# Wells-Group/pmg-dolfinx

Measured on NVIDIA B200. Metric: fine-level Gdof/s per p-MG V-cycle (P4->P2->P1, Chebyshev(2), CSR coarse solve), higher is better.
Workload: dtype f64

## Files before the change

pmg_dolfinx_b200/csrc/amg.cu:

```cuda
#include "common.hpp"
#include "operator.hpp"
#include "csr.hpp"
#include "solvers.hpp"
#include "amg.hpp"

#include <algorithm>
#include <cstdlib>
#include <cstring>

namespace pmgx
{
namespace
{
__global__ void __launch_bounds__(256)
k_dense_rows(int n_rows, int n_cols, const double* __restrict__ inv, const double* __restrict__ b,
             double* __restrict__ x)
{
  const int row = (blockIdx.x * blockDim.x + threadIdx.x) >> 5, lane = threadIdx.x & 31;
  if (row >= n_rows)
    return;
  const double* r = inv + (size_t)row * n_cols;
  double s = 0.0;
  for (int c = lane; c < n_cols; c += 32)
    s = fma(r[c], b[c], s);
#pragma unroll
  for (int o = 16; o > 0; o >>= 1)
    s += __shfl_xor_sync(0xffffffffu, s, o);
  if (lane == 0)
    x[row] = s;
}

__global__ void k_permute(int n, const int32_t* __restrict__ perm, const double* __restrict__ in, double* __restrict__ out)
{
  const int g = blockIdx.x * blockDim.x + threadIdx.x;
  if (g < n)
    out[g] = in[perm[g]];
}

struct RectSell
{
  int n_rows = 0;
  DevBuf<long long> slice_ptr;
  DevBuf<int32_t> cols;
  DevBuf<double> vals;
  void upload(const amg::Csr& M, cudaStream_t st)
  {
    n_rows = M.n_rows;
    const int ns = (n_rows + 31) / 32;
    std::vector<long long> sp((size_t)ns + 1, 0);
    for (int s = 0; s < ns; ++s)
    {
      int w = 0;
      for (int r = s * 32; r < std::min(n_rows, s * 32 + 32); ++r)
        w = std::max(w, (int)(M.ptr[r + 1] - M.ptr[r]));
      sp[s + 1] = sp[s] + (long long)w * 32;
    }
    std::vector<int32_t> c((size_t)std::max<long long>(sp[ns], 1), 0);
    std::vector<double> v((size_t)std::max<long long>(sp[ns], 1), 0.0);
    for (int r = 0; r < n_rows; ++r)
      for (int32_t j = M.ptr[r], k = 0; j < M.ptr[r + 1]; ++j, ++k)
      {
        const size_t p = (size_t)sp[r >> 5] + (size_t)k * 32 + (r & 31);
        c[p] = M.cols[j];
        v[p] = M.vals[j];
      }
    slice_ptr.upload(sp.data(), sp.size(), st);
    cols.upload(c.data(), c.size(), st);
    vals.upload(v.data(), v.size(), st);
  }
};

struct RectCsr
{
  int n_rows = 0;
  DevBuf<int32_t> ptr, cols;
  DevBuf<double> vals;
  void upload(const amg::Csr& M, cudaStream_t st)
  {
    n_rows = M.n_rows;
    ptr.upload(M.ptr.data(), M.ptr.size(), st);
    cols.upload(M.cols.data(), M.cols.size(), st);
    vals.upload(M.vals.data(), M.vals.size(), st);
  }
};

pmgx_halo* make_halo(pmgx_ctx* c, int n_owned, int n_ghost, const amg::Plan& p)
{
  if (c->nranks == 1)
    return nullptr;
  pmgx_halo* h = nullptr;
  const int rc = pmgx_halo_create(c, n_owned, n_ghost, (int)p.send_ranks.size(), p.send_ranks.data(), p.send_offsets.data(),
                                  p.send_idx.data(), (int)p.recv_ranks.size(), p.recv_ranks.data(), p.recv_offsets.data(),
                                  p.recv_idx.data(), &h);
  if (rc != PMGX_OK)
    throw Error{rc};
  static const bool ss = !(getenv("PMGX_AMG_SINGLE_STREAM") && atoi(getenv("PMGX_AMG_SINGLE_STREAM")) == 0);
  h->single_stream = ss && h->p2p && h->n_send() + h->n_recv() <= 65536;
  return h;
}

struct AmgPrecond : Precond
{
  struct Lv
  {
    int n_owned = 0, n_ghost = 0;
    long long nnz = 0;
    pmgx_operator* A = nullptr;
    bool own_A = false;
    pmgx_operator* A_lp = nullptr;
    pmgx_halo* halo = nullptr;
    pmgx_halo* halo_v = nullptr;
    pmgx_cheb* sm = nullptr;
    RectCsr R;
    RectSell P;
    DevBuf<double> x, b;
    DevBuf<double> x2, r2;
    long long nnz_p = 0;
    bool dense = false;
    int n_global = 0;
    DevBuf<double> inv;
    pmgx_halo* gather = nullptr;
    bool repl_first = false;
    int n_mine = 0;
    pmgx_halo* repl_gather = nullptr;
    DevBuf<double> bg;
    DevBuf<int32_t> perm;
  };
  pmgx_ctx* ctx = nullptr;
  std::vector<Lv> lv;
  int nu = 2;
  int gamma = 1;
  int gamma_from = 0;

  ~AmgPrecond() override
  {
    for (Lv& L : lv)
    {
      if (L.sm)
        pmgx_cheb_destroy(L.sm);
      if (L.A_lp)
        pmgx_operator_destroy(L.A_lp);
      if (L.own_A && L.A)
        pmgx_operator_destroy(L.A);
      if (L.halo)
        pmgx_halo_destroy(L.halo);
      if (L.gather)
        pmgx_halo_destroy(L.gather);
      if (L.repl_gather)
        pmgx_halo_destroy(L.repl_gather);
    }
  }

  void cycle(int l, const double* b, double* x)
  {
    Lv& L = lv[l];
    if (l + 1 == (int)lv.size())
    {
      if (L.dense)
      {
        double* bb = L.b.p;
        if (b != bb)
          vec::copy(ctx, bb, b, L.n_owned);
        if (L.gather)
        {
          halo_fwd_begin(L.gather, bb);
          halo_fwd_end(L.gather, bb);
        }
        if (L.n_owned > 0)
        {
          k_dense_rows<<<(L.n_owned * 32 + 255) / 256, 256, 0, ctx->stream>>>(L.n_owned, L.n_global, L.inv.p, bb, x);
          check_launch("k_dense_rows");
          count_launch(ctx);
        }
      }
      else
        cheb_solve(L.sm, L.A, x, b, nullptr, true, CHEB_R_NONE);
      return;
    }
    Lv& C = lv[l + 1];
    pmgx_operator* As = L.A_lp ? L.A_lp : L.A;
    cheb_solve(L.sm, As, x, b, nullptr, true, CHEB_R_FULL);
    if (L.halo_v)
    {
      halo_fwd_begin(L.halo_v, L.sm->r.p);
      halo_fwd_end(L.halo_v, L.sm->r.p);
    }
    if (C.repl_first)
    {
      spmv_rect(ctx, C.n_mine, L.R.ptr.p, L.R.cols.p, L.R.vals.p, L.sm->r.p, C.bg.p, false, 32);
      halo_fwd_begin(C.repl_gather, C.bg.p);
      halo_fwd_end(C.repl_gather, C.bg.p);
      k_permute<<<(C.n_owned + 255) / 256, 256, 0, ctx->stream>>>(C.n_owned, C.perm.p, C.bg.p, C.b.p);
      check_launch("k_permute");
      count_launch(ctx);
    }
    else
      spmv_rect(ctx, C.n_owned, L.R.ptr.p, L.R.cols.p, L.R.vals.p, L.sm->r.p, C.b.p, false, 32);
    cycle(l + 1, C.b.p, C.x.p);
    if (gamma == 2 && l >= gamma_from && l + 2 < (int)lv.size())
    {
      C.A->apply(C.x.p, C.r2.p);
      vec::axpy(ctx, C.r2.p, -1.0, C.r2.p, C.b.p, C.n_owned);
      cycle(l + 1, C.r2.p, C.x2.p);
      vec::axpy(ctx, C.x.p, 1.0, C.x2.p, C.x.p, C.n_owned);
    }
    if (C.halo_v)
    {
      halo_fwd_begin(C.halo_v, C.x.p);
      halo_fwd_end(C.halo_v, C.x.p);
    }
    spmv_sell_rect(ctx, L.n_owned, L.P.slice_ptr.p, L.P.cols.p, L.P.vals.p, C.x.p, x, true);
    cheb_solve(L.sm, As, x, b, nullptr, false, CHEB_R_NONE);
  }

  void apply(const double* r, double* u) override { cycle(0, r, u); }
};

amg::Plan plan_of(pmgx_halo* h)
{
  amg::Plan p;
  if (!h)
    return p;
  p.send_ranks = h->send_ranks;
  p.send_offsets = h->send_offsets;
  p.recv_ranks = h->recv_ranks;
  p.recv_offsets = h->recv_offsets;
  if (p.send_offsets.empty())
    p.send_offsets.assign(1, 0);
  if (p.recv_offsets.empty())
    p.recv_offsets.assign(1, 0);
  p.send_idx.resize((size_t)h->n_send());
  p.recv_idx.resize((size_t)h->n_recv());
  if (!p.send_idx.empty())
    PMGX_CUDA(cudaMemcpy(p.send_idx.data(), h->send_idx.p, p.send_idx.size() * sizeof(int32_t), cudaMemcpyDeviceToHost));
  if (!p.recv_idx.empty())
    PMGX_CUDA(cudaMemcpy(p.recv_idx.data(), h->recv_idx.p, p.recv_idx.size() * sizeof(int32_t), cudaMemcpyDeviceToHost));
  return p;
}
}
}

using pmgx::AmgPrecond;

extern "C"
{
int pmgx_coarse_create_amg(pmgx_ctx* ctx, pmgx_operator* A, int max_iter, double rtol, int nu, int min_coarse,
                           int max_levels, pmgx_coarse** out)
{
  PMGX_API_BEGIN
  PMGX_REQUIRE(ctx && A && out && max_iter >= 0, "coarse_create_amg: bad arguments");
  PMGX_REQUIRE(A->kind == pmgx_operator::CSR, "coarse_create_amg: the operator must be an assembled CSR operator");
  PMGX_REQUIRE(nu >= 1 && nu <= 8, "coarse_create_amg: nu must be in 1..8");
  PMGX_CUDA(cudaSetDevice(ctx->device));
  if (min_coarse <= 0)
    min_coarse = 600;
  if (max_levels <= 0)
    max_levels = 12;
  auto* Ac = static_cast<pmgx::CsrOperator*>(A);
  PMGX_REQUIRE(ctx->nranks == 1 || Ac->halo || Ac->n_ghost == 0, "coarse_create_amg: the operator has ghosts but no halo");
  pmgx::amg::Csr A0;
  A0.ptr.resize((size_t)Ac->n_owned + 1);
  A0.cols.resize((size_t)Ac->nnz);
  A0.vals.resize((size_t)Ac->nnz);
  {
    const int rc = pmgx_csr_get(A, A0.ptr.data(), A0.cols.data(), A0.vals.data());
    if (rc != PMGX_OK)
      return rc;
    std::vector<std::pair<int32_t, double>> row;
    for (int i = 0; i < Ac->n_owned; ++i)
    {
      bool sorted = true;
      for (int32_t j = A0.ptr[i] + 1; j < A0.ptr[i + 1] && sorted; ++j)
        sorted = A0.cols[j - 1] < A0.cols[j];
      if (sorted)
        continue;
      row.clear();
      for (int32_t j = A0.ptr[i]; j < A0.ptr[i + 1]; ++j)
        row.emplace_back(A0.cols[j], A0.vals[j]);
      std::sort(row.begin(), row.end());
      for (size_t t = 0; t < row.size(); ++t)
        A0.cols[A0.ptr[i] + t] = row[t].first, A0.vals[A0.ptr[i] + t] = row[t].second;
    }
  }
  pmgx::amg::Csr Az;
  if (getenv("PMGX_AMG_DROP_ZEROS") && atoi(getenv("PMGX_AMG_DROP_ZEROS")) == 1 && Ac->n_owned > 0)
  {
    A0.n_rows = Ac->n_owned;
    A0.n_cols = Ac->n_owned + Ac->n_ghost;
    Az = pmgx::amg::drop_stored_zeros(A0);
    if (Az.nnz() * 5 > A0.nnz() * 4)
      Az = pmgx::amg::Csr();
  }
  const pmgx::amg::Plan plan0 = pmgx::plan_of(Ac->halo);
  pmgx::amg::Comm cm;
  cm.rank = ctx->rank;
  cm.nranks = ctx->nranks;
  cm.allgather = [ctx](const void* mine, size_t bytes, void* all)
  {
    std::vector<char> buf;
    pmgx::p2p::allgather_bytes(ctx, mine, bytes, buf);
    std::memcpy(all, buf.data(), bytes * (size_t)ctx->nranks);
  };
  pmgx::amg::Hierarchy H;
  pmgx::amg::setup(H, std::move(A0), Ac->n_owned, Ac->n_ghost, plan0, cm, min_coarse, max_levels);

  std::unique_ptr<AmgPrecond> M(new AmgPrecond());
  M->ctx = ctx;
  M->nu = nu;
  int nu_coarse = nu;
  if (const char* e = getenv("PMGX_AMG_NU_COARSE"))
    nu_coarse = std::min(std::max(atoi(e), 1), 8);
  if (const char* e = getenv("PMGX_AMG_GAMMA"))
    M->gamma = atoi(e) == 2 ? 2 : 1;
  if (const char* e = getenv("PMGX_AMG_GAMMA_FROM"))
    M->gamma_from = std::max(atoi(e), 0);
  const bool use_lp = !(getenv("PMGX_AMG_LP") && atoi(getenv("PMGX_AMG_LP")) == 0);
  const int fuse_from = getenv("PMGX_AMG_FUSE_FROM") ? atoi(getenv("PMGX_AMG_FUSE_FROM")) : 1;
  const int nl = (int)H.levels.size();
  M->lv.resize((size_t)nl);
  for (int l = 0; l < nl; ++l)
  {
    pmgx::amg::Level& L = H.levels[l];
    AmgPrecond::Lv& D = M->lv[l];
    D.n_owned = L.n_owned;
    D.n_ghost = L.n_ghost;
    D.nnz = L.A.nnz();
    const bool last = l + 1 == nl;
    if (l == 0)
    {
      D.A = A;
      D.halo_v = Ac->halo;
      if (!Az.ptr.empty())
      {
        std::vector<int32_t> off((size_t)Ac->n_owned);
        for (int i = 0; i < Ac->n_owned; ++i)
        {
          int32_t j = Az.ptr[i];
          while (j < Az.ptr[i + 1] && Az.cols[j] < Ac->n_owned)
            ++j;
          off[i] = j;
        }
        pmgx_operator* Acmp = nullptr;
        const int rc = pmgx_csr_create(ctx, Ac->n_owned, Ac->n_ghost, Az.ptr.data(), off.data(), Az.cols.data(),
                                       Az.vals.data(), Ac->halo, &Acmp);
        if (rc != PMGX_OK)
          return rc;
        D.A = Acmp;
        D.own_A = true;
      }
    }
    else
    {
      if (!L.replicated)
      {
        D.halo = pmgx::make_halo(ctx, L.n_owned, L.n_ghost, L.plan);
        D.halo_v = D.halo;
      }
      else if (L.n_mine > 0 || !L.gather_perm.empty())
      {
        D.repl_first = true;
        D.n_mine = L.n_mine;
        D.repl_gather = pmgx::make_halo(ctx, L.n_mine, L.n_owned - L.n_mine, L.repl_plan);
        D.bg.alloc((size_t)std::max(L.n_owned, 1));
        PMGX_CUDA(cudaMemsetAsync(D.bg.p, 0, (size_t)std::max(L.n_owned, 1) * sizeof(double), ctx->stream));
        D.perm.upload(L.gather_perm.data(), L.gather_perm.size(), ctx->stream);
      }
      std::vector<int32_t> off((size_t)L.n_owned);
      for (int i = 0; i < L.n_owned; ++i)
      {
        int32_t j = L.A.ptr[i];
        while (j < L.A.ptr[i + 1] && L.A.cols[j] < L.n_owned)
          ++j;
        off[i] = j;
      }
      const int rc = pmgx_csr_create(ctx, L.n_owned, L.n_ghost, L.A.ptr.data(), off.data(), L.A.cols.data(),
                                     L.A.vals.data(), D.halo, &D.A);
      if (rc != PMGX_OK)
        return rc;
      D.own_A = true;
      const size_t nt = (size_t)L.n_owned + L.n_ghost;
      for (auto* buf : {&D.x, &D.b, &D.x2, &D.r2})
      {
        buf->alloc(nt);
        if (nt > 0)
          PMGX_CUDA(cudaMemsetAsync(buf->p, 0, nt * sizeof(double), ctx->stream));
      }
    }
    {
      const int rc = pmgx_cheb_create(ctx, L.n_owned, L.n_ghost, 0.1 * L.lmax, L.lmax, &D.sm);
      if (rc != PMGX_OK)
        return rc;
      D.sm->max_iter = (last && !L.dense) ? 4 * nu : (l == 0 ? nu : nu_coarse);
      D.sm->fuse = l >= fuse_from;
    }
    if (l == 0 && !last && use_lp)
      D.A_lp = pmgx::make_lp(static_cast<pmgx::CsrOperator*>(D.A));
    D.nnz_p = L.P.nnz();
    if (!last)
    {
      D.P.upload(L.P, ctx->stream);
      D.R.upload(L.R, ctx->stream);
    }
    else if (L.dense)
    {
      D.dense = true;
      D.n_global = (int)L.n_global;
      D.inv.upload(L.inv_rows.data(), L.inv_rows.size(), ctx->stream);
      const int n_gather = (int)L.n_global - L.n_owned;
      if (!L.replicated)
        D.gather = pmgx::make_halo(ctx, L.n_owned, n_gather, L.gather_plan);
      const size_t nt = (size_t)L.n_owned + std::max(L.n_ghost, n_gather);
      D.b.alloc(nt);
      if (nt > 0)
        PMGX_CUDA(cudaMemsetAsync(D.b.p, 0, nt * sizeof(double), ctx->stream));
    }
  }
  PMGX_CUDA(cudaStreamSynchronize(ctx->stream));

  pmgx_coarse* cs = nullptr;
  const int rc = pmgx_coarse_create(ctx, M->lv[0].A, max_iter, rtol, &cs);
  if (rc != PMGX_OK)
    return rc;
  cs->M = M.release();
  cs->check_every = 1;
  if (const char* e = getenv("PMGX_COARSE_CHECK_EVERY"))
    cs->check_every = std::max(atoi(e), 1);
  *out = cs;
  PMGX_API_END
}

int pmgx_coarse_num_levels(pmgx_coarse* cs)
{
  if (!cs)
    return -1;
  return cs->M ? (int)static_cast<AmgPrecond*>(cs->M)->lv.size() : 1;
}

int pmgx_coarse_level_info(pmgx_coarse* cs, int level, long long* out_h)
{
  PMGX_API_BEGIN
  PMGX_REQUIRE(cs && out_h && level >= 0 && level < pmgx_coarse_num_levels(cs), "coarse_level_info: bad arguments");
  if (!cs->M)
  {
    out_h[0] = cs->A->n_owned;
    out_h[1] = pmgx_csr_nnz(cs->A);
    out_h[2] = cs->A->n_ghost;
    out_h[3] = 0;
    out_h[4] = 0;
  }
  else
  {
    const AmgPrecond::Lv& L = static_cast<AmgPrecond*>(cs->M)->lv[level];
    out_h[0] = L.n_owned;
    out_h[1] = L.nnz;
    out_h[2] = L.n_ghost;
    out_h[3] = L.dense ? 1 : 0;
    out_h[4] = L.nnz_p;
  }
  PMGX_API_END
}

int pmgx_coarse_apply_preconditioner(pmgx_coarse* cs, const double* r, double* u)
{
  PMGX_API_BEGIN
  PMGX_REQUIRE(cs && r && u && r != u, "coarse_apply_preconditioner: bad arguments");
  PMGX_CUDA(cudaSetDevice(cs->ctx->device));
  if (cs->M)
    cs->M->apply(r, u);
  else
    pmgx::vec::pointwise_mult(cs->ctx, u, r, cs->A->diag_inv.p, cs->A->n_owned);
  PMGX_API_END
}
}
```

pmg_dolfinx_b200/csrc/csr.cu:

```cuda
#include "common.hpp"
#include "operator.hpp"
#include "csr.hpp"
#include "solvers.hpp"

namespace pmgx
{
namespace
{
constexpr int LPR = 8;
constexpr int ST = 256;

constexpr int UNR = 4;
template <bool ACCUM>
__global__ void __launch_bounds__(ST)
k_spmv(int n_rows, const double* __restrict__ vals, const int32_t* __restrict__ beg,
       const int32_t* __restrict__ end, const int32_t* __restrict__ cols,
       const double* __restrict__ x, double* __restrict__ y)
{
  const int gt = blockIdx.x * blockDim.x + threadIdx.x;
  const int row = gt / LPR, lane = gt % LPR;
  double s = 0.0;
  if (row < n_rows)
  {
    const int e = end[row];
    for (int j0 = beg[row] + lane; j0 < e; j0 += UNR * LPR)
    {
      int c[UNR];
      double v[UNR];
#pragma unroll
      for (int t = 0; t < UNR; ++t)
      {
        const int jj = j0 + t * LPR;
        const bool ok = jj < e;
        c[t] = ok ? __ldcs(cols + jj) : -1;
        v[t] = ok ? __ldcs(vals + jj) : 0.0;
      }
#pragma unroll
      for (int t = 0; t < UNR; ++t)
        if (c[t] >= 0)
          s = fma(v[t], x[c[t]], s);
    }
  }
#pragma unroll
  for (int o = LPR / 2; o > 0; o >>= 1)
    s += __shfl_xor_sync(0xffffffffu, s, o);
  if (row < n_rows && lane == 0)
    y[row] = ACCUM ? y[row] + s : s;
}

__global__ void __launch_bounds__(ST)
k_spmv_ghost_rows(int n_list, const int32_t* __restrict__ rows, const double* __restrict__ vals,
                  const int32_t* __restrict__ off_diag, const int32_t* __restrict__ row_ptr,
                  const int32_t* __restrict__ cols, const double* __restrict__ x, double* __restrict__ y)
{
  const int gt = blockIdx.x * blockDim.x + threadIdx.x;
  const int li = gt / LPR, lane = gt % LPR;
  double s = 0.0;
  int row = -1;
  if (li < n_list)
  {
    row = rows[li];
    const int e = row_ptr[row + 1];
    for (int j = off_diag[row] + lane; j < e; j += LPR)
      s = fma(vals[j], x[cols[j]], s);
  }
#pragma unroll
  for (int o = LPR / 2; o > 0; o >>= 1)
    s += __shfl_xor_sync(0xffffffffu, s, o);
  if (row >= 0 && lane == 0)
    y[row] += s;
}

template <int MODE>
__device__ __forceinline__ void cheb_row(int i, double q, const double* __restrict__ in, const ChebEp& e)
{
  if (MODE == ChebEp::INIT)
  {
    const double rv = q * (-1.0) + e.b[i];
    e.r[i] = rv;
    e.z_out[i] = (rv * e.dinv[i]) * e.c0;
  }
  else if (MODE == ChebEp::LAST)
    e.r[i] = q * (-1.0) + e.r[i];
  else
  {
    const double rv = q * (-1.0) + e.r[i];
    const double zo = in[i];
    const double zs = zo * e.c1;
    const double zv = (rv * e.dinv[i]) * e.c2 + zs;
    if (MODE == ChebEp::STEP)
    {
      e.r[i] = rv;
      e.z_out[i] = zv;
    }
    const double xo = e.defer == 2 ? zo : (e.defer == 1 ? zo * 1.0 + e.x[i] : e.x[i]);
    e.x[i] = zv * 1.0 + xo;
  }
}

template <typename VT, bool D16, int MODE>
__global__ void __launch_bounds__(ST)
k_spmv_cheb(int n_rows, const VT* __restrict__ vals, const int32_t* __restrict__ beg, const int32_t* __restrict__ end,
            const int32_t* __restrict__ row_ptr, const int16_t* __restrict__ dcol, const int32_t* __restrict__ cols,
            const double* __restrict__ x, const ChebEp e)
{
  const int gt = blockIdx.x * blockDim.x + threadIdx.x;
  const int row = gt / LPR, lane = gt % LPR;
  double s = 0.0;
  if (row < n_rows)
  {
    const int en = end[row];
    for (int j0 = beg[row] + lane; j0 < en; j0 += UNR * LPR)
    {
      int c[UNR];
      VT v[UNR];
#pragma unroll
      for (int t = 0; t < UNR; ++t)
      {
        const int jj = j0 + t * LPR;
        const bool ok = jj < en;
        c[t] = ok ? (D16 ? row + (int)__ldcs(dcol + jj) : __ldcs(cols + jj)) : -1;
        v[t] = ok ? __ldcs(vals + jj) : VT(0);
      }
#pragma unroll
      for (int t = 0; t < UNR; ++t)
        if (c[t] >= 0)
          s = fma((double)v[t], x[c[t]], s);
    }
  }
#pragma unroll
  for (int o = LPR / 2; o > 0; o >>= 1)
    s += __shfl_xor_sync(0xffffffffu, s, o);
  __shared__ double sq[ST / LPR];
  if (lane == 0)
    sq[threadIdx.x / LPR] = s;
  __syncthreads();
  if (threadIdx.x < ST / LPR)
  {
    const int r = blockIdx.x * (ST / LPR) + threadIdx.x;
    if (r < n_rows)
    {
      if (end[r] < row_ptr[r + 1])
        e.scratch[r] = sq[threadIdx.x];
      else
        cheb_row<MODE>(r, sq[threadIdx.x], x, e);
    }
  }
}

template <int MODE>
__global__ void __launch_bounds__(ST)
k_spmv_cheb_ghost_rows(int n_list, const int32_t* __restrict__ rows, const double* __restrict__ vals,
                       const int32_t* __restrict__ off_diag, const int32_t* __restrict__ row_ptr,
                       const int32_t* __restrict__ cols, const double* __restrict__ x, const ChebEp e)
{
  const int gt = blockIdx.x * blockDim.x + threadIdx.x;
  const int li = gt / LPR, lane = gt % LPR;
  double s = 0.0;
  int row = -1;
  if (li < n_list)
  {
    row = rows[li];
    const int en = row_ptr[row + 1];
    for (int j = off_diag[row] + lane; j < en; j += LPR)
      s = fma(vals[j], x[cols[j]], s);
  }
#pragma unroll
  for (int o = LPR / 2; o > 0; o >>= 1)
    s += __shfl_xor_sync(0xffffffffu, s, o);
  if (row >= 0 && lane == 0)
    cheb_row<MODE>(row, e.scratch[row] + s, x, e);
}

template <typename VT, bool D16>
void launch_spmv_cheb(pmgx_ctx* c, int grid, int n_rows, const VT* vals, const int32_t* beg, const int32_t* end,
                      const int32_t* row_ptr, const int16_t* dcol, const int32_t* cols, const double* x, const ChebEp& e)
{
  switch (e.mode)
  {
  case ChebEp::INIT: k_spmv_cheb<VT, D16, ChebEp::INIT><<<grid, ST, 0, c->stream>>>(n_rows, vals, beg, end, row_ptr, dcol, cols, x, e); break;
  case ChebEp::STEP: k_spmv_cheb<VT, D16, ChebEp::STEP><<<grid, ST, 0, c->stream>>>(n_rows, vals, beg, end, row_ptr, dcol, cols, x, e); break;
  case ChebEp::LAST: k_spmv_cheb<VT, D16, ChebEp::LAST><<<grid, ST, 0, c->stream>>>(n_rows, vals, beg, end, row_ptr, dcol, cols, x, e); break;
  default: k_spmv_cheb<VT, D16, ChebEp::XONLY><<<grid, ST, 0, c->stream>>>(n_rows, vals, beg, end, row_ptr, dcol, cols, x, e); break;
  }
  check_launch("k_spmv_cheb");
  count_launch(c);
}

void launch_ghost_rows_cheb(const CsrOperator* A, const double* x, const ChebEp& e)
{
  pmgx_ctx* c = A->ctx;
  const int g2 = (int)(((long long)A->n_ghost_rows * LPR + ST - 1) / ST);
#define PMGX_GR(M)                                                                                                     \
  k_spmv_cheb_ghost_rows<M><<<g2, ST, 0, c->stream>>>(A->n_ghost_rows, A->ghost_rows.p, A->values.p, A->off_diag.p,    \
                                                      A->row_ptr.p, A->cols.p, x, e)
  switch (e.mode)
  {
  case ChebEp::INIT: PMGX_GR(ChebEp::INIT); break;
  case ChebEp::STEP: PMGX_GR(ChebEp::STEP); break;
  case ChebEp::LAST: PMGX_GR(ChebEp::LAST); break;
  default: PMGX_GR(ChebEp::XONLY); break;
  }
#undef PMGX_GR
  check_launch("k_spmv_cheb_ghost_rows");
  count_launch(c);
}

__global__ void k_flag_ghost_rows(int n_rows, const int32_t* __restrict__ off_diag,
                                  const int32_t* __restrict__ row_ptr, int32_t* __restrict__ count,
                                  int32_t* __restrict__ list)
{
  const int i = blockIdx.x * blockDim.x + threadIdx.x;
  if (i < n_rows && off_diag[i] < row_ptr[i + 1])
    list[atomicAdd(count, 1)] = i;
}

__global__ void k_extract_diag_inv(int n_rows, const double* __restrict__ vals,
                                   const int32_t* __restrict__ row_ptr,
                                   const int32_t* __restrict__ cols, double* __restrict__ dinv)
{
  const int i = blockIdx.x * blockDim.x + threadIdx.x;
  if (i >= n_rows)
    return;
  double d = 0.0;
  for (int j = row_ptr[i]; j < row_ptr[i + 1]; ++j)
    if (cols[j] == i)
      d = 1.0 / vals[j];
  dinv[i] = d;
}

constexpr int SLICE = 32;

template <bool D16>
__global__ void __launch_bounds__(ST)
k_spmv_sell(int n_rows, const long long* __restrict__ slice_ptr, const float* __restrict__ vals,
            const int16_t* __restrict__ dcol, const int32_t* __restrict__ cols, const double* __restrict__ x,
            double* __restrict__ y)
{
  const int row = blockIdx.x * blockDim.x + threadIdx.x;
  const int s = row >> 5, lane = row & 31;
  if (s >= (n_rows + SLICE - 1) / SLICE)
    return;
  const long long b = slice_ptr[s];
  const int w = (int)((slice_ptr[s + 1] - b) >> 5);
  const float* v = vals + b + lane;
  const int16_t* d = dcol + b + lane;
  const int32_t* c = cols + b + lane;
  const int r = row < n_rows ? row : n_rows - 1;
  double s0 = 0.0, s1 = 0.0;
  int k = 0;
  for (; k + 4 <= w; k += 4)
  {
    float vv[4];
    int cc[4];
#pragma unroll
    for (int t = 0; t < 4; ++t)
    {
      vv[t] = __ldcs(v + (k + t) * SLICE);
      cc[t] = D16 ? r + (int)__ldcs(d + (k + t) * SLICE) : __ldcs(c + (k + t) * SLICE);
    }
    s0 = fma((double)vv[0], x[cc[0]], s0);
    s1 = fma((double)vv[1], x[cc[1]], s1);
    s0 = fma((double)vv[2], x[cc[2]], s0);
    s1 = fma((double)vv[3], x[cc[3]], s1);
  }
  for (; k < w; ++k)
  {
    const float vv = __ldcs(v + k * SLICE);
    const int cc = D16 ? r + (int)__ldcs(d + k * SLICE) : __ldcs(c + k * SLICE);
    s0 = fma((double)vv, x[cc], s0);
  }
  if (row < n_rows)
    y[row] = s0 + s1;
}

template <bool ACCUM>
__global__ void __launch_bounds__(ST)
k_spmv_sell_rect(int n_rows, const long long* __restrict__ slice_ptr, const double* __restrict__ vals,
                 const int32_t* __restrict__ cols, const double* __restrict__ x, double* __restrict__ y)
{
  const int row = blockIdx.x * blockDim.x + threadIdx.x;
  const int s = row >> 5, lane = row & 31;
  if (row >= n_rows)
    return;
  const long long b = slice_ptr[s];
  const int w = (int)((slice_ptr[s + 1] - b) >> 5);
  const double* v = vals + b + lane;
  const int32_t* c = cols + b + lane;
  double s0 = 0.0, s1 = 0.0;
  int k = 0;
  for (; k + 2 <= w; k += 2)
  {
    const double v0 = __ldcs(v + k * SLICE), v1 = __ldcs(v + (k + 1) * SLICE);
    const int c0 = __ldcs(c + k * SLICE), c1 = __ldcs(c + (k + 1) * SLICE);
    s0 = fma(v0, x[c0], s0);
    s1 = fma(v1, x[c1], s1);
  }
  if (k < w)
    s0 = fma(__ldcs(v + k * SLICE), x[__ldcs(c + k * SLICE)], s0);
  y[row] = ACCUM ? y[row] + (s0 + s1) : s0 + s1;
}

__global__ void k_sell_widths(int n_rows, const int32_t* __restrict__ row_ptr, const int32_t* __restrict__ off_diag,
                              const int32_t* __restrict__ cols, long long* __restrict__ widths, int* __restrict__ overflow)
{
  const int row = blockIdx.x * blockDim.x + threadIdx.x;
  int len = 0;
  bool ovf = false;
  if (row < n_rows)
  {
    len = off_diag[row] - row_ptr[row];
    for (int j = row_ptr[row]; j < off_diag[row]; ++j)
    {
      const int dlt = cols[j] - row;
      ovf = ovf || dlt > 32767 || dlt < -32767;
    }
  }
#pragma unroll
  for (int o = 16; o > 0; o >>= 1)
    len = max(len, __shfl_xor_sync(0xffffffffu, len, o));
  if (__any_sync(0xffffffffu, ovf) && (threadIdx.x & 31) == 0)
    atomicOr(overflow, 1);
  if ((threadIdx.x & 31) == 0 && row < n_rows)
    widths[row >> 5] = (long long)len * SLICE;
}

__global__ void k_sell_fill(int n_rows, const int32_t* __restrict__ row_ptr, const int32_t* __restrict__ off_diag,
                            const int32_t* __restrict__ cols, const double* __restrict__ vals,
                            const long long* __restrict__ slice_ptr, float* __restrict__ v32, int16_t* __restrict__ d16,
                            int32_t* __restrict__ c32)
{
  const int row = blockIdx.x * blockDim.x + threadIdx.x;
  const int s = row >> 5, lane = row & 31;
  if (s >= (n_rows + SLICE - 1) / SLICE)
    return;
  const long long b = slice_ptr[s];
  const int w = (int)((slice_ptr[s + 1] - b) >> 5);
  const int r = row < n_rows ? row : n_rows - 1;
  const int beg = row < n_rows ? row_ptr[row] : 0, len = row < n_rows ? off_diag[row] - row_ptr[row] : 0;
  for (int k = 0; k < w; ++k)
  {
    const long long p = b + (long long)k * SLICE + lane;
    const bool ok = k < len;
    v32[p] = ok ? (float)vals[beg + k] : 0.f;
    const int col = ok ? cols[beg + k] : r;
    if (d16)
      d16[p] = (int16_t)(col - r);
    if (c32)
      c32[p] = col;
  }
}

template <int LANES, bool ACCUM>
__global__ void __launch_bounds__(ST)
k_spmv_rect(int n_rows, const double* __restrict__ vals, const int32_t* __restrict__ ptr,
            const int32_t* __restrict__ cols, const double* __restrict__ x, double* __restrict__ y)
{
  const int gt = blockIdx.x * blockDim.x + threadIdx.x;
  const int row = gt / LANES, lane = gt % LANES;
  double s = 0.0;
  if (row < n_rows)
  {
    const int e = ptr[row + 1];
    for (int j = ptr[row] + lane; j < e; j += LANES)
      s = fma(vals[j], x[cols[j]], s);
  }
#pragma unroll
  for (int o = LANES / 2; o > 0; o >>= 1)
    s += __shfl_xor_sync(0xffffffffu, s, o);
  if (row < n_rows && lane == 0)
    y[row] = ACCUM ? y[row] + s : s;
}
}

void spmv_sell_rect(pmgx_ctx* c, int n_rows, const long long* slice_ptr, const int32_t* cols, const double* vals,
                    const double* x, double* y, bool accumulate)
{
  if (n_rows <= 0)
    return;
  const int grid = (n_rows + ST - 1) / ST;
  if (accumulate)
    k_spmv_sell_rect<true><<<grid, ST, 0, c->stream>>>(n_rows, slice_ptr, vals, cols, x, y);
  else
    k_spmv_sell_rect<false><<<grid, ST, 0, c->stream>>>(n_rows, slice_ptr, vals, cols, x, y);
  check_launch("k_spmv_sell_rect");
  count_launch(c);
}

void spmv_rect(pmgx_ctx* c, int n_rows, const int32_t* row_ptr, const int32_t* cols, const double* vals,
               const double* x, double* y, bool accumulate, int lanes)
{
  if (n_rows <= 0)
    return;
  const int grid = (int)(((long long)n_rows * lanes + ST - 1) / ST);
  if (lanes == 32)
  {
    if (accumulate)
      k_spmv_rect<32, true><<<grid, ST, 0, c->stream>>>(n_rows, vals, row_ptr, cols, x, y);
    else
      k_spmv_rect<32, false><<<grid, ST, 0, c->stream>>>(n_rows, vals, row_ptr, cols, x, y);
  }
  else if (lanes == 4)
  {
    if (accumulate)
      k_spmv_rect<4, true><<<grid, ST, 0, c->stream>>>(n_rows, vals, row_ptr, cols, x, y);
    else
      k_spmv_rect<4, false><<<grid, ST, 0, c->stream>>>(n_rows, vals, row_ptr, cols, x, y);
  }
  else
  {
    if (accumulate)
      k_spmv_rect<8, true><<<grid, ST, 0, c->stream>>>(n_rows, vals, row_ptr, cols, x, y);
    else
      k_spmv_rect<8, false><<<grid, ST, 0, c->stream>>>(n_rows, vals, row_ptr, cols, x, y);
  }
  check_launch("k_spmv_rect");
  count_launch(c);
}

void CsrOperator::apply(double* x, double* y)
{
  cudaSetDevice(ctx->device);
  const int grid = (int)(((long long)n_owned * LPR + ST - 1) / ST);
  if (n_ghost > 0)
    vec::set(ctx, y + n_owned, n_ghost, 0.0);
  if (halo)
    halo_fwd_begin(halo, x);
  if (n_owned > 0)
  {
    k_spmv<false><<<grid, ST, 0, ctx->stream>>>(n_owned, values.p, row_ptr.p, off_diag.p, cols.p, x, y);
    check_launch("k_spmv");
    count_launch(ctx);
  }
  if (halo)
    halo_fwd_end(halo, x);
  if (n_ghost_rows > 0)
  {
    const int g2 = (int)(((long long)n_ghost_rows * LPR + ST - 1) / ST);
    k_spmv_ghost_rows<<<g2, ST, 0, ctx->stream>>>(n_ghost_rows, ghost_rows.p, values.p, off_diag.p, row_ptr.p, cols.p,
                                                  x, y);
    check_launch("k_spmv_ghost_rows");
    count_launch(ctx);
  }
}

bool CsrOperator::apply_cheb(double* in, const ChebEp& e)
{
  cudaSetDevice(ctx->device);
  PMGX_REQUIRE(n_ghost_rows == 0 || e.scratch, "apply_cheb: scratch vector missing");
  const int grid = (int)(((long long)n_owned * LPR + ST - 1) / ST);
  if (halo)
    halo_fwd_begin(halo, in);
  if (n_owned > 0)
    launch_spmv_cheb<double, false>(ctx, grid, n_owned, values.p, row_ptr.p, off_diag.p, row_ptr.p, nullptr, cols.p, in, e);
  if (halo)
    halo_fwd_end(halo, in);
  if (n_ghost_rows > 0)
    launch_ghost_rows_cheb(this, in, e);
  return true;
}

void CsrOperatorLP::apply(double* x, double* y)
{
  cudaSetDevice(ctx->device);
  if (n_ghost > 0)
    vec::set(ctx, y + n_owned, n_ghost, 0.0);
  if (halo)
    halo_fwd_begin(halo, x);
  if (n_owned > 0)
  {
    const int grid = (n_slices * SLICE + ST - 1) / ST;
    if (d16)
      k_spmv_sell<true><<<grid, ST, 0, ctx->stream>>>(n_owned, slice_ptr.p, vals32.p, dcol16.p, nullptr, x, y);
    else
      k_spmv_sell<false><<<grid, ST, 0, ctx->stream>>>(n_owned, slice_ptr.p, vals32.p, nullptr, cols32.p, x, y);
    check_launch("k_spmv_sell");
    count_launch(ctx);
  }
  if (halo)
    halo_fwd_end(halo, x);
  if (src->n_ghost_rows > 0)
  {
    const int g2 = (int)(((long long)src->n_ghost_rows * LPR + ST - 1) / ST);
    k_spmv_ghost_rows<<<g2, ST, 0, ctx->stream>>>(src->n_ghost_rows, src->ghost_rows.p, src->values.p, src->off_diag.p,
                                                  src->row_ptr.p, src->cols.p, x, y);
    check_launch("k_spmv_ghost_rows");
    count_launch(ctx);
  }
}

CsrOperatorLP* make_lp(CsrOperator* A)
{
  pmgx_ctx* c = A->ctx;
  std::unique_ptr<CsrOperatorLP> L(new CsrOperatorLP());
  L->ctx = c;
  L->kind = pmgx_operator::CSR;
  L->n_owned = A->n_owned;
  L->n_ghost = A->n_ghost;
  L->halo = A->halo;
  L->src = A;
  L->diag_inv.alloc((size_t)A->n_owned);
  if (A->n_owned > 0)
    PMGX_CUDA(cudaMemcpyAsync(L->diag_inv.p, A->diag_inv.p, (size_t)A->n_owned * sizeof(double), cudaMemcpyDeviceToDevice, c->stream));
  const int n = A->n_owned;
  L->n_slices = (n + SLICE - 1) / SLICE;
  L->slice_ptr.alloc((size_t)L->n_slices + 1);
  PMGX_CUDA(cudaMemsetAsync(L->slice_ptr.p, 0, ((size_t)L->n_slices + 1) * sizeof(long long), c->stream));
  DevBuf<int> ovf;
  ovf.alloc(1);
  PMGX_CUDA(cudaMemsetAsync(ovf.p, 0, sizeof(int), c->stream));
  long long total = 0;
  if (n > 0)
  {
    k_sell_widths<<<(n + ST - 1) / ST, ST, 0, c->stream>>>(n, A->row_ptr.p, A->off_diag.p, A->cols.p, L->slice_ptr.p + 1, ovf.p);
    check_launch("k_sell_widths");
    std::vector<long long> sp((size_t)L->n_slices + 1, 0);
    PMGX_CUDA(cudaMemcpyAsync(sp.data(), L->slice_ptr.p, sp.size() * sizeof(long long), cudaMemcpyDeviceToHost, c->stream));
    PMGX_CUDA(cudaStreamSynchronize(c->stream));
    for (size_t i = 1; i < sp.size(); ++i)
      sp[i] += sp[i - 1];
    total = sp.back();
    PMGX_CUDA(cudaMemcpyAsync(L->slice_ptr.p, sp.data(), sp.size() * sizeof(long long), cudaMemcpyHostToDevice, c->stream));
    PMGX_CUDA(cudaStreamSynchronize(c->stream));
  }
  int o = 0;
  PMGX_CUDA(cudaMemcpyAsync(&o, ovf.p, sizeof(int), cudaMemcpyDeviceToHost, c->stream));
  PMGX_CUDA(cudaStreamSynchronize(c->stream));
  L->d16 = o == 0;
  const size_t cap = (size_t)std::max<long long>(total, 1);
  L->vals32.alloc(cap);
  if (L->d16)
    L->dcol16.alloc(cap);
  else
    L->cols32.alloc(cap);
  if (n > 0)
  {
    k_sell_fill<<<(L->n_slices * SLICE + ST - 1) / ST, ST, 0, c->stream>>>(n, A->row_ptr.p, A->off_diag.p, A->cols.p, A->values.p,
                                                                         L->slice_ptr.p, L->vals32.p, L->dcol16.p, L->cols32.p);
    check_launch("k_sell_fill");
    PMGX_CUDA(cudaStreamSynchronize(c->stream));
  }
  return L.release();
}

void CsrOperator::finish_setup()
{
  n_ghost_rows = 0;
  if (n_owned > 0 && has_ghost_cols)
  {
    DevBuf<int32_t> count;
    count.alloc(1);
    ghost_rows.alloc((size_t)n_owned);
    PMGX_CUDA(cudaMemsetAsync(count.p, 0, sizeof(int32_t), ctx->stream));
    k_flag_ghost_rows<<<(n_owned + 255) / 256, 256, 0, ctx->stream>>>(n_owned, off_diag.p, row_ptr.p, count.p,
                                                                      ghost_rows.p);
    check_launch("k_flag_ghost_rows");
    PMGX_CUDA(cudaMemcpyAsync(&n_ghost_rows, count.p, sizeof(int32_t), cudaMemcpyDeviceToHost, ctx->stream));
    PMGX_CUDA(cudaStreamSynchronize(ctx->stream));
  }
  diag_inv.alloc((size_t)n_owned);
  if (n_owned > 0)
  {
    k_extract_diag_inv<<<(n_owned + 255) / 256, 256, 0, ctx->stream>>>(n_owned, values.p, row_ptr.p,
                                                                       cols.p, diag_inv.p);
    check_launch("k_extract_diag_inv");
    count_launch(ctx);
    PMGX_CUDA(cudaStreamSynchronize(ctx->stream));
  }
}
}

using pmgx::CsrOperator;

extern "C"
{
int pmgx_csr_create(pmgx_ctx* ctx, int n_rows, int n_ghost, const int32_t* row_ptr_h,
                    const int32_t* off_diag_offset_h, const int32_t* cols_h, const double* values_h,
                    pmgx_halo* halo, pmgx_operator** out)
{
  PMGX_API_BEGIN
  PMGX_REQUIRE(ctx && out && row_ptr_h, "csr_create: null argument");
  PMGX_REQUIRE(n_rows >= 0 && n_ghost >= 0, "csr_create: bad sizes");
  PMGX_CUDA(cudaSetDevice(ctx->device));
  const long long nnz = row_ptr_h[n_rows];
  PMGX_REQUIRE(row_ptr_h[0] == 0 && nnz >= 0, "csr_create: bad row_ptr");
  bool ghost_cols = false;
  for (int i = 0; i < n_rows; ++i)
  {
    PMGX_REQUIRE(row_ptr_h[i] <= off_diag_offset_h[i] && off_diag_offset_h[i] <= row_ptr_h[i + 1],
                 "csr_create: off_diag_offset outside its row");
    ghost_cols = ghost_cols || off_diag_offset_h[i] < row_ptr_h[i + 1];
  }
  for (long long j = 0; j < nnz; ++j)
    PMGX_REQUIRE(cols_h[j] >= 0 && cols_h[j] < n_rows + n_ghost, "csr_create: column out of range");
  std::unique_ptr<CsrOperator> A(new CsrOperator());
  A->ctx = ctx;
  A->kind = pmgx_operator::CSR;
  A->n_owned = n_rows;
  A->n_ghost = n_ghost;
  A->halo = halo;
  A->nnz = nnz;
  A->has_ghost_cols = ghost_cols;
  A->row_ptr.upload(row_ptr_h, (size_t)n_rows + 1, ctx->stream);
  A->off_diag.upload(off_diag_offset_h, (size_t)n_rows, ctx->stream);
  A->cols.upload(cols_h, (size_t)nnz, ctx->stream);
  A->values.upload(values_h, (size_t)nnz, ctx->stream);
  A->finish_setup();
  *out = A.release();
  PMGX_API_END
}

long long pmgx_csr_nnz(pmgx_operator* op)
{
  if (!op || op->kind != pmgx_operator::CSR)
    return -1;
  return static_cast<CsrOperator*>(op)->nnz;
}

int pmgx_csr_get(pmgx_operator* op, int32_t* row_ptr_h, int32_t* cols_h, double* values_h)
{
  PMGX_API_BEGIN
  PMGX_REQUIRE(op && op->kind == pmgx_operator::CSR, "csr_get: not a CSR operator");
  auto* A = static_cast<CsrOperator*>(op);
  PMGX_CUDA(cudaSetDevice(A->ctx->device));
  PMGX_CUDA(cudaStreamSynchronize(A->ctx->stream));
  if (row_ptr_h)
    PMGX_CUDA(cudaMemcpy(row_ptr_h, A->row_ptr.p, ((size_t)A->n_owned + 1) * sizeof(int32_t), cudaMemcpyDeviceToHost));
  if (cols_h && A->nnz > 0)
    PMGX_CUDA(cudaMemcpy(cols_h, A->cols.p, (size_t)A->nnz * sizeof(int32_t), cudaMemcpyDeviceToHost));
  if (values_h && A->nnz > 0)
    PMGX_CUDA(cudaMemcpy(values_h, A->values.p, (size_t)A->nnz * sizeof(double), cudaMemcpyDeviceToHost));
  PMGX_API_END
}
}
```

pmg_dolfinx_b200/csrc/csr.hpp:

```cpp
#pragma once
#include "operator.hpp"

namespace pmgx
{
struct CsrOperator : pmgx_operator
{
  long long nnz = 0;
  bool has_ghost_cols = false;
  DevBuf<int32_t> row_ptr;
  DevBuf<int32_t> off_diag;
  DevBuf<int32_t> cols;
  DevBuf<double> values;
  DevBuf<int32_t> ghost_rows;
  int n_ghost_rows = 0;
  void apply(double* x, double* y) override;
  bool supports_cheb_fusion() const override { return true; }
  bool apply_cheb(double* in, const ChebEp& e) override;
  void finish_setup();
};

struct CsrOperatorLP : pmgx_operator
{
  CsrOperator* src = nullptr;
  bool d16 = false;
  int n_slices = 0;
  DevBuf<long long> slice_ptr;
  DevBuf<float> vals32;
  DevBuf<int16_t> dcol16;
  DevBuf<int32_t> cols32;
  void apply(double* x, double* y) override;
};
CsrOperatorLP* make_lp(CsrOperator* A);
}
```

Measured before the change: 4.827.

## Fuse Chebyshev update into SELL low-precision SpMV and drop stored zeros by default

Adds a fused SELL-format float-value SpMV kernel that applies the Chebyshev smoother update per row, so the low-precision operator can take part in smoother fusion. Fusion now defaults to starting at level 0. Stored zeros are now always dropped from the coarse operator and from the P and R transfer matrices. Together these aim to cut kernel launches and memory traffic in the AMG coarse solve, at the cost of more template instantiations and an always-on zero-drop pass during setup.

```diff
diff --git a/pmg_dolfinx_b200/csrc/amg.cu b/pmg_dolfinx_b200/csrc/amg.cu
--- a/pmg_dolfinx_b200/csrc/amg.cu
+++ b/pmg_dolfinx_b200/csrc/amg.cu
@@ -283,7 +283,7 @@
     }
   }
   pmgx::amg::Csr Az;
-  if (getenv("PMGX_AMG_DROP_ZEROS") && atoi(getenv("PMGX_AMG_DROP_ZEROS")) == 1 && Ac->n_owned > 0)
+  if (Ac->n_owned > 0)
   {
     A0.n_rows = Ac->n_owned;
     A0.n_cols = Ac->n_owned + Ac->n_ghost;
@@ -315,7 +315,7 @@
   if (const char* e = getenv("PMGX_AMG_GAMMA_FROM"))
     M->gamma_from = std::max(atoi(e), 0);
   const bool use_lp = !(getenv("PMGX_AMG_LP") && atoi(getenv("PMGX_AMG_LP")) == 0);
-  const int fuse_from = getenv("PMGX_AMG_FUSE_FROM") ? atoi(getenv("PMGX_AMG_FUSE_FROM")) : 1;
+  const int fuse_from = getenv("PMGX_AMG_FUSE_FROM") ? atoi(getenv("PMGX_AMG_FUSE_FROM")) : 0;
   const int nl = (int)H.levels.size();
   M->lv.resize((size_t)nl);
   for (int l = 0; l < nl; ++l)
@@ -398,8 +398,8 @@
     D.nnz_p = L.P.nnz();
     if (!last)
     {
-      D.P.upload(L.P, ctx->stream);
-      D.R.upload(L.R, ctx->stream);
+      D.P.upload(pmgx::amg::drop_stored_zeros(L.P), ctx->stream);
+      D.R.upload(pmgx::amg::drop_stored_zeros(L.R), ctx->stream);
     }
     else if (L.dense)
     {
diff --git a/pmg_dolfinx_b200/csrc/csr.cu b/pmg_dolfinx_b200/csrc/csr.cu
--- a/pmg_dolfinx_b200/csrc/csr.cu
+++ b/pmg_dolfinx_b200/csrc/csr.cu
@@ -232,15 +232,11 @@
 constexpr int SLICE = 32;
 
 template <bool D16>
-__global__ void __launch_bounds__(ST)
-k_spmv_sell(int n_rows, const long long* __restrict__ slice_ptr, const float* __restrict__ vals,
-            const int16_t* __restrict__ dcol, const int32_t* __restrict__ cols, const double* __restrict__ x,
-            double* __restrict__ y)
-{
-  const int row = blockIdx.x * blockDim.x + threadIdx.x;
+__device__ __forceinline__ double sell_row(int row, int n_rows, const long long* __restrict__ slice_ptr,
+                                           const float* __restrict__ vals, const int16_t* __restrict__ dcol,
+                                           const int32_t* __restrict__ cols, const double* __restrict__ x)
+{
   const int s = row >> 5, lane = row & 31;
-  if (s >= (n_rows + SLICE - 1) / SLICE)
-    return;
   const long long b = slice_ptr[s];
   const int w = (int)((slice_ptr[s + 1] - b) >> 5);
   const float* v = vals + b + lane;
@@ -270,8 +266,40 @@
     const int cc = D16 ? r + (int)__ldcs(d + k * SLICE) : __ldcs(c + k * SLICE);
     s0 = fma((double)vv, x[cc], s0);
   }
+  return s0 + s1;
+}
+
+template <bool D16>
+__global__ void __launch_bounds__(ST)
+k_spmv_sell(int n_rows, const long long* __restrict__ slice_ptr, const float* __restrict__ vals,
+            const int16_t* __restrict__ dcol, const int32_t* __restrict__ cols, const double* __restrict__ x,
+            double* __restrict__ y)
+{
+  const int row = blockIdx.x * blockDim.x + threadIdx.x;
+  if ((row >> 5) >= (n_rows + SLICE - 1) / SLICE)
+    return;
+  const double s = sell_row<D16>(row, n_rows, slice_ptr, vals, dcol, cols, x);
   if (row < n_rows)
-    y[row] = s0 + s1;
+    y[row] = s;
+}
+
+template <bool D16, int MODE>
+__global__ void __launch_bounds__(ST)
+k_spmv_sell_cheb(int n_rows, const long long* __restrict__ slice_ptr, const float* __restrict__ vals,
+                 const int16_t* __restrict__ dcol, const int32_t* __restrict__ cols,
+                 const int32_t* __restrict__ off_diag, const int32_t* __restrict__ row_ptr,
+                 const double* __restrict__ x, const ChebEp e)
+{
+  const int row = blockIdx.x * blockDim.x + threadIdx.x;
+  if ((row >> 5) >= (n_rows + SLICE - 1) / SLICE)
+    return;
+  const double s = sell_row<D16>(row, n_rows, slice_ptr, vals, dcol, cols, x);
+  if (row >= n_rows)
+    return;
+  if (off_diag && off_diag[row] < row_ptr[row + 1])
+    e.scratch[row] = s;
+  else
+    cheb_row<MODE>(row, s, x, e);
 }
 
 template <bool ACCUM>
@@ -460,6 +488,30 @@
   return true;
 }
 
+namespace
+{
+template <bool D16>
+void launch_sell_cheb(const CsrOperatorLP* L, const double* x, const ChebEp& e)
+{
+  const CsrOperator* A = L->src;
+  const int grid = (L->n_slices * SLICE + ST - 1) / ST;
+  const int32_t* od = A->n_ghost_rows > 0 ? A->off_diag.p : nullptr;
+#define PMGX_SC(M)                                                                                                     \
+  k_spmv_sell_cheb<D16, M><<<grid, ST, 0, L->ctx->stream>>>(L->n_owned, L->slice_ptr.p, L->vals32.p, L->dcol16.p,       \
+                                                            L->cols32.p, od, A->row_ptr.p, x, e)
+  switch (e.mode)
+  {
+  case ChebEp::INIT: PMGX_SC(ChebEp::INIT); break;
+  case ChebEp::STEP: PMGX_SC(ChebEp::STEP); break;
+  case ChebEp::LAST: PMGX_SC(ChebEp::LAST); break;
+  default: PMGX_SC(ChebEp::XONLY); break;
+  }
+#undef PMGX_SC
+  check_launch("k_spmv_sell_cheb");
+  count_launch(L->ctx);
+}
+}
+
 void CsrOperatorLP::apply(double* x, double* y)
 {
   cudaSetDevice(ctx->device);
@@ -487,6 +539,26 @@
     check_launch("k_spmv_ghost_rows");
     count_launch(ctx);
   }
+}
+
+bool CsrOperatorLP::apply_cheb(double* in, const ChebEp& e)
+{
+  cudaSetDevice(ctx->device);
+  PMGX_REQUIRE(src->n_ghost_rows == 0 || e.scratch, "apply_cheb: scratch vector missing");
+  if (halo)
+    halo_fwd_begin(halo, in);
+  if (n_owned > 0)
+  {
+    if (d16)
+      launch_sell_cheb<true>(this, in, e);
+    else
+      launch_sell_cheb<false>(this, in, e);
+  }
+  if (halo)
+    halo_fwd_end(halo, in);
+  if (src->n_ghost_rows > 0)
+    launch_ghost_rows_cheb(src, in, e);
+  return true;
 }
 
 CsrOperatorLP* make_lp(CsrOperator* A)
diff --git a/pmg_dolfinx_b200/csrc/csr.hpp b/pmg_dolfinx_b200/csrc/csr.hpp
--- a/pmg_dolfinx_b200/csrc/csr.hpp
+++ b/pmg_dolfinx_b200/csrc/csr.hpp
@@ -29,6 +29,8 @@
   DevBuf<int16_t> dcol16;
   DevBuf<int32_t> cols32;
   void apply(double* x, double* y) override;
+  bool supports_cheb_fusion() const override { return true; }
+  bool apply_cheb(double* in, const ChebEp& e) override;
 };
 CsrOperatorLP* make_lp(CsrOperator* A);
 }
```

Measured after the change: 5.411, median of 6. 1.12x the previous value.
